# alehdaghi/vq-vae-2-pytorch

Hardware: AMD Instinct MI355X
Metric: images/sec VQ-VAE-2 256px train step (higher is better)
Workload: dtype f32; 1 GPU; configs[1]: 256x256 FFHQ-shaped synthetic, default two-level VQ-VAE-2, batch 32/GPU; global_batch=32, image=256, n_embed=512, parallelism=dp1

## Files before the change

### include/vq2.h

```cpp
#ifndef VQ2_H
#define VQ2_H

#include <stddef.h>
#include <stdint.h>

#ifdef __cplusplus
extern "C" {
#endif

#define VQ2_OK 0
#define VQ2_ERR_INVALID 1
#define VQ2_ERR_UNSUPPORTED 2
#define VQ2_ERR_WORKSPACE 3
#define VQ2_ERR_LAUNCH 4

typedef void *vq2_stream_t;

#define VQ2_API_VERSION 12

int vq2_version(void);
const char *vq2_last_error(void);

int vq2_prof_enable(int level);
int vq2_prof_report(char *buf, size_t cap);

typedef struct vq2_conv_desc {
    int32_t N, H, W, Ci;
    int32_t Co;
    int32_t KH, KW, stride, pad;
    int32_t transposed;
    int32_t ldx, ldy;
    int32_t Cir, Cor;
} vq2_conv_desc;

#define VQ2_RELU_IN 1
#define VQ2_RELU_OUT 2

#define VQ2_PACK_FWD 0
#define VQ2_PACK_DGRAD 1
int vq2_pack_weight(const vq2_conv_desc *d, int which, const float *w, float *packed, vq2_stream_t stream);

typedef struct vq2_pack_job {
    const float *w;
    float *packed;
    int64_t offset;
    int64_t numel;
    int32_t Or, Ir, Op, Ip, KH, KW, mode, reserved;
} vq2_pack_job;
int vq2_pack_job_init(const vq2_conv_desc *d, int which, const float *w, float *packed, vq2_pack_job *job);
int vq2_pack_weights_batched(const vq2_pack_job *jobs_dev, int32_t njobs, int64_t total, vq2_stream_t stream);

// ... 7 lines not shown

size_t vq2_resblock_w2_workspace_bytes(int32_t N, int32_t H, int32_t W, int32_t C, int32_t Cm);
int vq2_resblock_bwd_data(int32_t N, int32_t H, int32_t W, int32_t C, int32_t Cm, const float *g, int32_t ldg,
                          const float *r, int32_t ldr, const float *x, int32_t ldx, const float *w2d, const float *w1d,
                          float *dh, int32_t lddh, float *dx, int32_t lddx, void *w2_ws, vq2_stream_t stream);

int vq2_conv_dgrad(const vq2_conv_desc *d, const float *dy, const float *wp, const float *mask, int32_t ldmask,
                   const float *residual, int32_t ldres, float *dx, int32_t lddx, vq2_stream_t stream);
#define VQ2_MASK_AFTER_RESIDUAL 4
int vq2_conv_dgrad_ex(const vq2_conv_desc *d, int flags, const float *dy, const float *wp, const float *mask,
                      int32_t ldmask, const float *residual, int32_t ldres, float *dx, int32_t lddx,
                      vq2_stream_t stream);

size_t vq2_conv_wgrad_workspace_bytes(const vq2_conv_desc *d);
int vq2_conv_wgrad(const vq2_conv_desc *d, int flags, const float *x, const float *dy, float *dw, float *db, void *ws,
                   size_t ws_bytes, vq2_stream_t stream);

typedef struct vq2_wgrad_job {
    const float *ws;
    float *dw;
    const float *bias_ws;
    float *db;
    int64_t unit_offset;
    int32_t O, I, Or, Ir, taps, S, n_units_w, n_units_b;
    int32_t swapped;
    int32_t bias_splits;
} vq2_wgrad_job;
int vq2_conv_wgrad_partial(const vq2_conv_desc *d, int flags, const float *x, const float *dy, float *db, void *ws,
                           size_t ws_bytes, vq2_stream_t stream);
int vq2_wgrad_job_init(const vq2_conv_desc *d, const void *ws, float *dw, float *db, vq2_wgrad_job *job);
int vq2_wgrad_reduce_batched(const vq2_wgrad_job *jobs_dev, int32_t njobs, int64_t total_units, vq2_stream_t stream);
int vq2_resblock_w2_job_init(int32_t N, int32_t H, int32_t W, int32_t C, int32_t Cm, const void *ws, float *dw, float *db,
                             vq2_wgrad_job *job);

size_t vq2_colsum_workspace_bytes(int64_t rows, int32_t C);
int vq2_colsum(const float *dy, int64_t rows, int32_t C, int32_t ld, float *db, void *ws, size_t ws_bytes,
               vq2_stream_t stream);

int vq2_nchw_to_nhwc(const float *src, float *dst, int32_t N, int32_t C, int32_t H, int32_t W, int32_t ld,
                     vq2_stream_t stream);
int vq2_nhwc_to_nchw(const float *src, float *dst, int32_t N, int32_t C, int32_t H, int32_t W, int32_t ld,
                     vq2_stream_t stream);

#define VQ2_U8_HWC 0
#define VQ2_U8_CHW 1
int vq2_u8_to_nhwc4(const uint8_t *src, int layout, int32_t N, int32_t C, int32_t Hs, int32_t Ws, int32_t y0,
                    int32_t x0, int32_t H, int32_t W, const float *lut ,
                    float *dst , vq2_stream_t stream);
int vq2_nhwc_to_u8(const float *src, int32_t ld, int32_t N, int32_t C, int32_t H, int32_t W,
                   const float *inv_s , const float *mean , uint8_t *dst, int layout,
                   int32_t Hc, int32_t Wc, int64_t pitch, int32_t cols, int32_t pad, int64_t image_pitch, vq2_stream_t stream);
int vq2_relu_bwd(const float *dy, int32_t lddy, const float *y, int32_t ldy, float *g, int32_t ldg, int64_t pixels,
                 int32_t C, vq2_stream_t stream);
int vq2_slice_copy(const float *src, int32_t lds, float *dst, int32_t ldd, int64_t pixels, int32_t C,
                   int accumulate, vq2_stream_t stream);

int vq2_vq_prepare(const float *embed, float *embedT, float *enorm, int32_t D, int32_t K, vq2_stream_t stream);
size_t vq2_vq_fwd_workspace_floats(int64_t M, int32_t D, int32_t K);
int vq2_vq_fwd(const float *x, int32_t ldx, const float *embed, const float *embedT, const float *enorm, int64_t M,
               int32_t D, int32_t K, int64_t *idx, float *out, int32_t ldo, float *ws, vq2_stream_t stream);
size_t vq2_vq_stats_workspace_bytes(int64_t M, int32_t D, int32_t K);
int vq2_vq_stats(const float *x, int32_t ldx, const int64_t *idx, int64_t M, int32_t D, int32_t K, float *counts,
                 float *sumsT, void *ws, size_t ws_bytes, vq2_stream_t stream);
int vq2_vq_loss(const float *loss_partial, int64_t M, int32_t D, float *diff, vq2_stream_t stream);
int vq2_vq_bwd(const float *g_out, int32_t ldg, const float *g_diff, const float *x, int32_t ldx,
               const int64_t *idx, const float *embedT, int64_t M, int32_t D, int32_t K, float *dx, int32_t lddx,
// ... 158 lines not shown
```

### vq-vae-2-pytorch_amd/_lib.py

```python
import ctypes as C
import os

_HERE = os.path.dirname(os.path.abspath(__file__))
LIB_PATH = os.environ.get("VQ2_LIB") or os.path.join(_HERE, "libvq2.so")

c_f32p = C.c_void_p
c_stream = C.c_void_p


class ConvDesc(C.Structure):
    _fields_ = [(n, C.c_int32) for n in
                ("N", "H", "W", "Ci", "Co", "KH", "KW", "stride", "pad", "transposed", "ldx", "ldy", "Cir", "Cor")]


class ConvGeom(C.Structure):
    _fields_ = [(n, C.c_int32) for n in
                ("N", "H", "W", "Ci", "Co", "KH", "KW", "pad_top", "pad_left", "ldx", "ldy", "Cir", "Cor", "reserved")]


class PackJob(C.Structure):
    _fields_ = [("w", C.c_void_p), ("packed", C.c_void_p), ("offset", C.c_int64), ("numel", C.c_int64)] + \
               [(n, C.c_int32) for n in ("Or", "Ir", "Op", "Ip", "KH", "KW", "mode", "reserved")]


# ... 15 lines not shown

class WnEntry(C.Structure):
    _fields_ = [("v_off", C.c_int64), ("g_off", C.c_int64), ("w_off", C.c_int64)] + \
               [(n, C.c_int32) for n in ("rows", "cols", "kh", "kw", "mask_from", "row_start")]


def _load():
    if not os.path.exists(LIB_PATH):
        raise ImportError(
            f"{LIB_PATH} not found: build it with `python -c 'import __graft_entry__ as g; g.build()'` "
            "(vq-vae-2-pytorch_amd/csrc/build.sh).  There is no CPU or eager fallback for this path.")
    import torch
    lib = C.CDLL(LIB_PATH)
    P, I32, I64, SZ, F, D = C.c_void_p, C.c_int32, C.c_int64, C.c_size_t, C.c_float, C.c_double
    DP = C.POINTER(ConvDesc)
    GP = C.POINTER(ConvGeom)
    U64 = C.c_uint64
    sig = {
        "vq2_version": (C.c_int, []),
        "vq2_last_error": (C.c_char_p, []),
        "vq2_prof_enable": (C.c_int, [C.c_int]),
        "vq2_prof_report": (C.c_int, [C.c_char_p, SZ]),
        "vq2_pack_weight": (C.c_int, [DP, C.c_int, P, P, P]),
        "vq2_pack_job_init": (C.c_int, [DP, C.c_int, P, P, C.POINTER(PackJob)]),
        "vq2_pack_weights_batched": (C.c_int, [P, I32, I64, P]),
        "vq2_conv_fwd": (C.c_int, [DP, C.c_int, P, P, P, P, I32, P, P]),
        "vq2_conv_dgrad": (C.c_int, [DP, P, P, P, I32, P, I32, P, I32, P]),
        "vq2_conv_dgrad_ex": (C.c_int, [DP, C.c_int, P, P, P, I32, P, I32, P, I32, P]),
        "vq2_conv_wgrad_workspace_bytes": (SZ, [DP]),
        "vq2_conv_wgrad": (C.c_int, [DP, C.c_int, P, P, P, P, P, SZ, P]),
        "vq2_conv_wgrad_partial": (C.c_int, [DP, C.c_int, P, P, P, P, SZ, P]),
        "vq2_wgrad_job_init": (C.c_int, [DP, P, P, P, C.POINTER(WgradJob)]),
        "vq2_wgrad_reduce_batched": (C.c_int, [P, I32, I64, P]),
        "vq2_colsum_workspace_bytes": (SZ, [I64, I32]),
        "vq2_colsum": (C.c_int, [P, I64, I32, I32, P, P, SZ, P]),
        "vq2_nchw_to_nhwc": (C.c_int, [P, P, I32, I32, I32, I32, I32, P]),
        "vq2_nhwc_to_nchw": (C.c_int, [P, P, I32, I32, I32, I32, I32, P]),
        "vq2_u8_to_nhwc4": (C.c_int, [P, C.c_int, I32, I32, I32, I32, I32, I32, I32, I32, P, P, P]),
        "vq2_nhwc_to_u8": (C.c_int, [P, I32, I32, I32, I32, I32, C.POINTER(F), C.POINTER(F), P, C.c_int, I32, I32, I64, I32,
                                     I32, I64, P]),
        "vq2_sse_workspace_bytes": (SZ, [I32, I32, I32, I32]),
        "vq2_sse_per_image": (C.c_int, [P, P, I32, I32, I32, I32, P, P, SZ, P]),
        "vq2_index_hist": (C.c_int, [P, I64, I32, P, P, P]),
        "vq2_eval_accumulate": (C.c_int, [P, I32, I64, P, P, P]),
        "vq2_image_metrics_workspace_bytes": (SZ, [I32, I32, I32, I32]),
        "vq2_image_metrics": (C.c_int, [P, I32, P, I32, I32, I32, I32, I32, C.POINTER(F), C.POINTER(F), P, P, P, SZ, P]),
        "vq2_image_metrics_accumulate": (C.c_int, [P, P, I32, P, P, P]),
        "vq2_relu_bwd": (C.c_int, [P, I32, P, I32, P, I32, I64, I32, P]),
        "vq2_resblock_supported": (C.c_int, [I32, I32]),
        "vq2_resblock_bwd_data": (C.c_int, [I32, I32, I32, I32, I32, P, I32, P, I32, P, I32, P, P, P, I32, P, I32, P, P]),
        "vq2_resblock_w2_workspace_bytes": (SZ, [I32, I32, I32, I32, I32]),
        "vq2_resblock_w2_job_init": (C.c_int, [I32, I32, I32, I32, I32, P, P, P, C.POINTER(WgradJob)]),
        "vq2_resblock_fwd": (C.c_int, [I32, I32, I32, I32, I32, C.c_int, P, I32, P, P, P, P, P, I32, P, I32, P]),
        "vq2_slice_copy": (C.c_int, [P, I32, P, I32, I64, I32, C.c_int, P]),
        "vq2_vq_prepare": (C.c_int, [P, P, P, I32, I32, P]),
        "vq2_vq_fwd_workspace_floats": (SZ, [I64, I32, I32]),
        "vq2_vq_fwd": (C.c_int, [P, I32, P, P, P, I64, I32, I32, P, P, I32, P, P]),
        "vq2_vq_stats_workspace_bytes": (SZ, [I64, I32, I32]),
        "vq2_vq_stats": (C.c_int, [P, I32, P, I64, I32, I32, P, P, P, SZ, P]),
        "vq2_vq_loss": (C.c_int, [P, I64, I32, P, P]),
        "vq2_vq_bwd": (C.c_int, [P, I32, P, P, I32, P, P, I64, I32, I32, P, I32, P]),
        "vq2_vq_ema_update": (C.c_int, [P, P, P, P, P, I32, I32, D, D, P, P]),
        "vq2_vq_ema_update_prepare": (C.c_int, [P, P, P, P, P, I32, I32, D, D, P, P, P, P]),
        "vq2_vq_gather": (C.c_int, [P, P, I64, I32, I32, P, I32, P]),
        "vq2_instnorm_stats": (C.c_int, [P, I32, I32, I64, I32, D, P, P, P]),
        "vq2_adain_fwd": (C.c_int, [P, I32, P, P, P, I32, I64, I32, C.c_int, P, I32, P]),
# ... 78 lines not shown
```

### vq-vae-2-pytorch_amd/csrc/vq2_wgrad.hip

```cpp
#include "vq2_conv.h"

namespace vq2 {

struct WgradParams {
    const float *x;
    const float *g;
    float *ws;
    float *bias_ws;
    int bias_taps;
    int bias_nslots;
    int N, H, W, I, ldx;
    int Ho, Wo, O, ldg;
    int KH, KW, stride, pad_h, pad_w;
    int K, M;
    int rows_per_split;
    int relu_x, relu_g;
};

constexpr int WG_BKR = 32;

constexpr int rows_per_pass(int c4) {
    int r = 32;
    while (r * c4 > 256) r >>= 1;
    return r;
// ... 648 lines not shown
        const int t = (is_bias ? lu - j.n_units_w : lu) * 32 + lane;
        float s0 = 0.f, s1 = 0.f, s2 = 0.f, s3 = 0.f;
        if (t < limit) {
            int z = g;
            for (; z + 24 < nsplit; z += 32) {
                s0 += src[(size_t)z * total + t];
                s1 += src[(size_t)(z + 8) * total + t];
                s2 += src[(size_t)(z + 16) * total + t];
                s3 += src[(size_t)(z + 24) * total + t];
            }
            for (; z < nsplit; z += 8) s0 += src[(size_t)z * total + t];
        }
        part[g][lane] = (s0 + s1) + (s2 + s3);
        __syncthreads();
        if (g == 0 && t < limit) {
            float s = part[0][lane];
#pragma unroll
            for (int q = 1; q < 8; ++q) s += part[q][lane];
            if (is_bias) {
                j.db[t] = s;
            } else {
                const int o = t / K, k = t - o * K;
                const int tap = k / j.I, i = k - tap * j.I;
                if (o < j.Or && i < j.Ir) {
                    if (j.swapped & 1) j.dw[((size_t)i * j.Or + o) * j.taps + (j.taps - 1 - tap)] = s;
                    else j.dw[((size_t)o * j.Ir + i) * j.taps + tap] = s;
                }
            }
        }
        __syncthreads();
    }
}

enum WgradRole { WGRAD_PLAIN, WGRAD_EXCHANGED, WGRAD_CONVT };
enum WgradFamily { WGRAD_GEN, WGRAD_FAST, WGRAD_WINO };

struct WgradPlan {
    int role, family;
    int wino;
    int tile;
    int O, I, K, M, S, rows_per_split;
    int Or, Ir;
    int bias_taps, bias_nslots, bias_splits;
    size_t bias_floats;
    int mode;
    long ext_x, ext_g;
};

static WgradParams wgrad_operands(const ConvGeo *d, int role) {
    WgradParams P{};
    P.N = d->N; P.KH = d->KH; P.KW = d->KW; P.stride = d->stride; P.pad_h = d->pad_h; P.pad_w = d->pad_w;
    P.H = d->H; P.W = d->W; P.Ho = d->H; P.Wo = d->W;
    P.ldx = role == WGRAD_PLAIN ? d->ldx : d->ldy;
    P.ldg = role == WGRAD_PLAIN ? d->ldy : d->ldx;
    if (role == WGRAD_PLAIN) { P.Ho = out_hw(d).h; P.Wo = out_hw(d).w; }
    else if (role == WGRAD_CONVT) { P.H = 2 * d->H; P.W = 2 * d->W; }
    else { P.stride = 1; P.pad_h = P.pad_w = d->KH - 1 - d->pad_h; }
    return P;
}

template <int WM, int WN, int MT, int NT>
static int launch_wgrad(const WgradPlan &pl, const WgradParams &P, hipStream_t s) {
    constexpr int BMO = WM * MT * 32, BNK = WN * NT * 32;
    const bool rx = P.relu_x, rg = P.relu_g;
    void (*kern)(const WgradParams) = nullptr;
    if (pl.family == WGRAD_GEN) kern = wgrad_kernel<WM, WN, MT, NT>;
    else if (pl.family == WGRAD_FAST)
        kern = rx ? wgrad_fast_kernel<WM, WN, MT, NT, true, false>
                  : rg ? wgrad_fast_kernel<WM, WN, MT, NT, false, true> : wgrad_fast_kernel<WM, WN, MT, NT, false, false>;
    else if constexpr (BMO == 128 && BNK == 128) {
        if (pl.wino == 1) kern = rx ? wgrad_fast_kernel<WM, WN, MT, NT, true, false, 1> : wgrad_fast_kernel<WM, WN, MT, NT, false, false, 1>;
        if (pl.wino == 2)
            kern = rx ? wgrad_fast_kernel<WM, WN, MT, NT, true, false, 2>
                      : rg ? wgrad_fast_kernel<WM, WN, MT, NT, false, true, 2> : wgrad_fast_kernel<WM, WN, MT, NT, false, false, 2>;
    } else if constexpr (BMO == 128 && BNK == 96) {
        if (pl.wino == 3) kern = rg ? wgrad_fast_kernel<WM, WN, MT, NT, false, true, 3> : wgrad_fast_kernel<WM, WN, MT, NT, false, false, 3>;
    }
    if (!kern) return set_error(VQ2_ERR_INVALID, "conv_wgrad: the %d x %d tile has no Winograd mode %d", BMO, BNK, pl.wino);
    const size_t lds = (size_t)2 * WG_BKR * (BMO + BNK) * sizeof(float);
// ... 69 lines not shown
            if (best < 0 || work < best) { best = work; p.tile = c; }
        }
    }
    if (wino && p.role == WGRAD_EXCHANGED && d->KH == 3 && d->pad_h == 1 && p.I == 32 && p.O % 128 == 0 &&
        (d->W % 64 == 0 || (d->W == 32 && d->H % 2 == 0))) {
        p.wino = 3;
        p.K = 4 * 96;
        p.M = p.M / 2;
        p.tile = wgrad_tile_of(128, 96);
    }
    const int bmo = WGRAD_TILES[p.tile].bmo, bnk = WGRAD_TILES[p.tile].bnk;
    const int tiles = ((p.K + bnk - 1) / bnk) * ((p.O + bmo - 1) / bmo);
    const int lds = 2 * WG_BKR * (bmo + bnk) * 4;
    int per_cu = (160 * 1024) / lds;
    if (per_cu > 4) per_cu = 4;
    int S = (256 * per_cu) / tiles;
    const int max_s = (p.M + 255) / 256;
    if (S > max_s) S = max_s;
    if (S < 1) S = 1;
    int rps = (p.M + S - 1) / S;
    rps = (rps + 31) / 32 * 32;
    p.S = (p.M + rps - 1) / rps;
    p.rows_per_split = rps;
    p.ext_x = (long)d->N * v.H * v.W * v.ldx;
    p.ext_g = (long)p.M * v.ldg;
    const bool fast_ok = fast && v.Wo % WG_BKR == 0 && p.rows_per_split % WG_BKR == 0 && p.ext_x < FAST_REACH && p.ext_g < FAST_REACH;
    p.family = p.wino ? WGRAD_WINO : fast_ok ? WGRAD_FAST : WGRAD_GEN;
    if (p.wino == 2 && d->transposed) { p.bias_taps = 1; p.bias_nslots = 4; }
    else if (p.role == WGRAD_EXCHANGED) { p.bias_taps = 1 << ((d->KH / 2) * d->KW + d->KW / 2); p.bias_nslots = 1; }
    else if (d->transposed) { p.bias_taps = (1 << 5) | (1 << 6) | (1 << 9) | (1 << 10); p.bias_nslots = 4; }
    p.bias_floats = p.bias_taps ? (size_t)p.S * p.bias_nslots * p.I : (size_t)p.S * p.O;
    p.bias_splits = p.bias_taps ? p.S * p.bias_nslots : 0;
    p.mode = (p.role == WGRAD_EXCHANGED) | (p.wino << 1);
    return p;
}

static size_t wgrad_ws_bytes(const WgradPlan &p) { return ((size_t)p.S * p.O * p.K + p.bias_floats) * sizeof(float); }

static int wgrad_params(const ConvGeo *d, const WgradPlan &p, int flags, const float *x, const float *dy, float *db, void *ws,
                        WgradParams &P) {
    VQ2_REQUIRE(p.ext_x < (1L << 31) && p.ext_g < (1L << 31), "conv_wgrad: tensor exceeds 2^31 elements");
    const bool plain = p.role == WGRAD_PLAIN;
    const int relu = (flags & VQ2_RELU_IN) != 0;
    P = wgrad_operands(d, p.role);
    P.x = plain ? x : dy; P.relu_x = plain ? relu : 0;
    P.g = plain ? dy : x; P.relu_g = plain ? 0 : relu;
    P.ws = static_cast<float *>(ws);
    P.bias_ws = db ? P.ws + (size_t)p.S * p.O * p.K : nullptr;
    P.bias_taps = p.bias_taps; P.bias_nslots = p.bias_nslots;
    P.O = p.O; P.I = p.I; P.K = p.K; P.M = p.M; P.rows_per_split = p.rows_per_split;
    return VQ2_OK;
}

static const char *wgrad_label(const WgradPlan &p, const WgradTile &t, const ConvGeo *d) {
    const char *form = p.wino == 3 ? "swwino" : p.role == WGRAD_EXCHANGED ? "sw" : p.wino == 1 ? "wino" : p.wino == 2 ? "wino4" : "";
    return prof_label("wgrad<%dx%d>%s|O=%d,K=%d,M=%d,S=%d,k%d,%s", t.bmo, t.bnk, form, p.O, p.K, p.M, p.S, d->KH,
                      p.family == WGRAD_GEN ? "gen" : "fast");
}

constexpr int CS_MAX_BLOCKS = 512;

static inline int64_t cs_rows_per_block(int64_t rows) {
    int64_t rpb = (rows + CS_MAX_BLOCKS - 1) / CS_MAX_BLOCKS;
    return rpb < 256 ? 256 : rpb;
}

__global__ __launch_bounds__(256) void colsum_partial_kernel(const float *__restrict__ x, int64_t rows, int C, int ld,
                                                             int64_t rpb, float *__restrict__ part) {
    extern __shared__ __attribute__((aligned(16))) float red[];
    const int C4 = C / 4;
    const int nrg = 256 / C4 > 0 ? 256 / C4 : 1;
    const int64_t r0 = (int64_t)blockIdx.x * rpb;
    const int64_t r1 = r0 + rpb < rows ? r0 + rpb : rows;
    for (int cbase = 0; cbase < C4; cbase += 256) {
        const int c4 = cbase + (int)(threadIdx.x % (C4 < 256 ? C4 : 256));
        const int rg = threadIdx.x / (C4 < 256 ? C4 : 256);
        float4 a = make_float4(0.f, 0.f, 0.f, 0.f);
        if (rg < nrg && c4 < C4) {
            for (int64_t r = r0 + rg; r < r1; r += nrg) {
                const float4 v = *reinterpret_cast<const float4 *>(x + r * ld + c4 * 4);
                a.x += v.x; a.y += v.y; a.z += v.z; a.w += v.w;
            }
            *reinterpret_cast<float4 *>(red + (size_t)rg * C + c4 * 4) = a;
        }
        __syncthreads();
        for (int c = threadIdx.x; c < C; c += 256) {
            if (c / 4 >= cbase && c / 4 < cbase + 256) {
                float s = 0.f;
                for (int g = 0; g < nrg; ++g) s += red[(size_t)g * C + c];
                part[(size_t)blockIdx.x * C + c] = s;
// ... 99 lines not shown
    if (int e = wgrad_params(d, p, flags, x, dy, db, ws, P)) return e;
    hipStream_t s = to_stream(stream);
    const WgradTile &tile = WGRAD_TILES[p.tile];
    const ConvWork work = conv_work(d, 0, 0);
    ProfScope prof(prof_enabled() ? wgrad_label(p, tile, d) : "wgrad", work.flops, work.bytes, s);
    if (int e = tile.launch(p, P, s)) return e;
    if (!reduce) return VQ2_OK;
    vq2_wgrad_job j;
    wgrad_job_init_impl(d, p, ws, dw, db, &j);
    const int total = p.O * p.K;
    const int blocks = (total + 31) / 32 < 4096 ? (total + 31) / 32 : 4096;
    hipLaunchKernelGGL(wgrad_reduce_kernel, dim3(blocks), dim3(256), 0, s, j.ws, j.dw, j.O, j.I, j.Or, j.Ir, j.taps, j.S,
                       j.bias_ws, j.db, j.swapped, j.bias_splits);
    return check_launch("wgrad_reduce_kernel");
}

extern "C" int vq2_conv_wgrad(const vq2_conv_desc *d, int flags, const float *x, const float *dy, float *dw, float *db,
                              void *ws, size_t ws_bytes, vq2_stream_t stream) {
    return wgrad_impl(d, flags, x, dy, dw, db, ws, ws_bytes, stream, true);
}
extern "C" int vq2_conv_wgrad_partial(const vq2_conv_desc *d, int flags, const float *x, const float *dy, float *db,
                                      void *ws, size_t ws_bytes, vq2_stream_t stream) {
    return wgrad_impl(d, flags, x, dy, nullptr, db, ws, ws_bytes, stream, false);
}
extern "C" int vq2_convg_wgrad(const vq2_conv_geom *d, int flags, const float *x, const float *dy, float *dw, float *db,
                               void *ws, size_t ws_bytes, vq2_stream_t stream) {
    return wgrad_impl(d, flags, x, dy, dw, db, ws, ws_bytes, stream, true);
}
extern "C" int vq2_convg_wgrad_partial(const vq2_conv_geom *d, int flags, const float *x, const float *dy, float *db,
                                       void *ws, size_t ws_bytes, vq2_stream_t stream) {
    return wgrad_impl(d, flags, x, dy, nullptr, db, ws, ws_bytes, stream, false);
}

template <class Desc>
static int wgrad_job_entry(const Desc *d, const void *ws, float *dw, float *db, vq2_wgrad_job *job) {
    ConvGeo g;
    if (int e = entry_geo(d, "wgrad_job_init", g)) return e;
    VQ2_REQUIRE(ws && dw && job, "wgrad_job_init: null pointer");
    VQ2_REQUIRE(!g.same || (g.N > 0 && g.H > 0 && g.W > 0 && g.Ci > 0 && g.Co > 0), "wgrad_job_init: non-positive dims");
    if (int e = check_forms()) return e;
    wgrad_job_init_impl(&g, plan_wgrad(&g), ws, dw, db, job);
    return VQ2_OK;
}

extern "C" int vq2_wgrad_job_init(const vq2_conv_desc *d, const void *ws, float *dw, float *db, vq2_wgrad_job *job) {
    return wgrad_job_entry(d, ws, dw, db, job);
}
extern "C" int vq2_convg_wgrad_job_init(const vq2_conv_geom *d, const void *ws, float *dw, float *db, vq2_wgrad_job *job) {
    return wgrad_job_entry(d, ws, dw, db, job);
}

extern "C" int vq2_wgrad_reduce_batched(const vq2_wgrad_job *jobs_dev, int32_t njobs, int64_t total_units,
                                        vq2_stream_t stream) {
    VQ2_REQUIRE(jobs_dev && njobs > 0 && total_units > 0, "wgrad_reduce_batched: bad arguments");
    const unsigned blocks = (unsigned)(total_units < 8192 ? total_units : 8192);
    hipLaunchKernelGGL(wgrad_reduce_batched_kernel, dim3(blocks), dim3(256), 0, to_stream(stream), jobs_dev, njobs,
                       total_units);
    return check_launch("wgrad_reduce_batched_kernel");
}

extern "C" size_t vq2_colsum_workspace_bytes(int64_t rows, int32_t C) {
    if (rows <= 0 || C <= 0) return 0;
    const int64_t rpb = cs_rows_per_block(rows);
    return (size_t)((rows + rpb - 1) / rpb) * C * sizeof(float);
}

// ... 9 lines not shown
```

### vq-vae-2-pytorch_amd/ops.py

```python
from dataclasses import dataclass
from types import SimpleNamespace
import contextlib
import ctypes as C
import os

import torch
from torch.autograd import Function

from ._lib import lib, check, AttnDesc, ConvDesc, ConvGeom, OneHotDesc, PackJob, WgradJob, WnEntry

VQ2_RELU_IN = 1
VQ2_RELU_OUT = 2
VQ2_MASK_AFTER_RESIDUAL = 4
PACK_FWD = 0
PACK_DGRAD = 1



def _stream():
    return C.c_void_p(torch.cuda.current_stream().cuda_stream)


_THIS_STREAM = contextlib.nullcontext()

# ... 207 lines not shown
    check(_abi(spec).fwd(C.byref(d), flags, _p(x), _p(wp), _p(bias), _p(residual), ldres, _p(out), _stream()),
          "conv_fwd")
    return out


def conv_dgrad(spec, xshape, dy, weight, mask=None, residual=None, out=None, mask_after=False):
    n, h, w, _ = xshape
    if out is None:
        out = torch.empty((n, h, w, spec.ci), device=dy.device, dtype=torch.float32)
    d = _desc(spec, n, h, w, spec.ci, ld_of(dy))
    wp = packed_weight(spec, weight, PACK_DGRAD)
    check(_abi(spec).dgrad(C.byref(d), VQ2_MASK_AFTER_RESIDUAL if mask_after else 0, _p(dy), _p(wp), _p(mask),
                                ld_of(mask) if mask is not None else 0, _p(residual),
                                ld_of(residual) if residual is not None else 0, _p(out), ld_of(out), _stream()),
          "conv_dgrad")
    return out


def _grad_slot(param):
    slot = getattr(param, "_vq2_grad", None) if param is not None else None
    if slot is not None and (not param.is_leaf or param.grad is None):
        return slot.view_as(slot)
    return None if param is None else torch.empty_like(param, memory_format=torch.contiguous_format)


class WgradBatch:

    def __init__(self):
        self.entries = {}
        self.order = []
        self.tables = {}
        self.dirty = True

    def launch(self, spec, x, dy, relu_in, weight, bias, want_db, side):
        n, h, w, _ = x.shape
        key = (id(weight), n, h, w, ld_of(x), ld_of(dy), relu_in)
        d = _desc(spec, n, h, w, ld_of(x), ld_of(dy))
        ent = self.entries.get(key)
        if ent is None:
            nbytes = _abi(spec).wgrad_workspace_bytes(C.byref(d))
            ws = torch.empty(max(nbytes // 4, 4), device=x.device, dtype=torch.float32)
            dw = weight._vq2_grad
            db = bias._vq2_grad if (bias is not None and want_db) else None
            job = WgradJob()
            check(_abi(spec).wgrad_job_init(C.byref(d), _p(ws), _p(dw), _p(db), C.byref(job)), "wgrad_job_init")
            ent = {"ws": ws, "nbytes": nbytes, "job": job, "dw": dw, "db": db, "used": False}
            self.entries[key] = ent
            self.dirty = True
        on_side = n * h * w <= WGRAD_STREAM_MAX_PIXELS
        if on_side:
            side.wait_event(torch.cuda.current_stream().record_event())
        with (torch.cuda.stream(side) if on_side else _THIS_STREAM):
            check(_abi(spec).wgrad_partial(C.byref(d), VQ2_RELU_IN if relu_in else 0, _p(x), _p(dy), _p(ent["db"]),
                                             _p(ent["ws"]), ent["nbytes"], _stream()), "conv_wgrad_partial")
        if on_side:
            x.record_stream(side)
            dy.record_stream(side)
        if not ent["used"]:
            ent["used"] = True
            self.order.append(key)
        dw, db = ent["dw"], ent["db"]
        return dw.view_as(dw), (None if db is None else db.view_as(db))

    def resblock_w2(self, n, h, w, c, cm, weight, bias):
        key = (id(weight), n, h, w, "rbw2")
        ent = self.entries.get(key)
        if ent is None:
            nbytes = lib.vq2_resblock_w2_workspace_bytes(n, h, w, c, cm)
            ws = torch.empty(max(nbytes // 4, 4), device=weight.device, dtype=torch.float32)
            dw, db = weight._vq2_grad, bias._vq2_grad
            job = WgradJob()
            check(lib.vq2_resblock_w2_job_init(n, h, w, c, cm, _p(ws), _p(dw), _p(db), C.byref(job)), "resblock_w2_job_init")
            ent = {"ws": ws, "nbytes": nbytes, "job": job, "dw": dw, "db": db, "used": False}
            self.entries[key] = ent
            self.dirty = True
        if not ent["used"]:
            ent["used"] = True
            self.order.append(key)
        return ent["ws"], ent["dw"].view_as(ent["dw"]), ent["db"].view_as(ent["db"])

    def flush(self):
        if not self.order:
            return
        sig = tuple(self.order)
        if self.dirty:
            self.tables = {}
            self.dirty = False
        tab = self.tables.get(sig)
        if tab is None:
            import numpy as np
            arr = (WgradJob * len(self.order))()
            off = 0
            for i, key in enumerate(self.order):
                job = self.entries[key]["job"]
                job.unit_offset = off
                arr[i] = job
                off += job.n_units_w + job.n_units_b
            raw = np.frombuffer(bytes(arr), dtype=np.uint8).copy()
            tab = (torch.from_numpy(raw).to(self.entries[self.order[0]]["ws"].device), off)
            self.tables[sig] = tab
        check(lib.vq2_wgrad_reduce_batched(_p(tab[0]), len(self.order), tab[1], _stream()), "wgrad_reduce_batched")
        for key in self.order:
            self.entries[key]["used"] = False
        self.order = []


class StepContext:

    def __init__(self, wgrad_stream):
        self.batch = WgradBatch()
        self.stream = wgrad_stream
        self.active = False


def _step_ctx(weight):
    ctx = getattr(weight, "_vq2_ctx", None)
    return ctx if (ctx is not None and ctx.active) else None


WGRAD_STREAM_MAX_PIXELS = 40000


def conv_wgrad(spec, x, dy, relu_in, weight, bias=None, want_dw=True, want_db=True):
    n, h, w, _ = x.shape
    d = _desc(spec, n, h, w, ld_of(x), ld_of(dy))
    nbytes = _abi(spec).wgrad_workspace_bytes(C.byref(d))
    sc = _step_ctx(weight)
    if sc is not None and getattr(weight, "_vq2_grad", None) is not None and weight.grad is None and \
            (bias is None or (getattr(bias, "_vq2_grad", None) is not None and bias.grad is None)) and \
            (bias is None or bias.numel() == spec.cout):
        dw, db = sc.batch.launch(spec, x, dy, relu_in, weight, bias, want_db, sc.stream)
        return (dw if want_dw else None), db
    dw = _grad_slot(weight)
    db = _grad_slot(bias) if (bias is not None and want_db) else None
    side = None
    if sc is not None and getattr(weight, "_vq2_grad", None) is not None and dw.data_ptr() == weight._vq2_grad.data_ptr():
        side = sc.stream
        side.wait_event(torch.cuda.current_stream().record_event())
    with (torch.cuda.stream(side) if side is not None else _THIS_STREAM):
        ws = torch.empty(max(nbytes // 4, 4), device=x.device, dtype=torch.float32)
        check(_abi(spec).wgrad(C.byref(d), VQ2_RELU_IN if relu_in else 0, _p(x), _p(dy), _p(dw), _p(db), _p(ws), nbytes,
                                 _stream()), "conv_wgrad")
    if side is not None:
        x.record_stream(side)
        dy.record_stream(side)
    return (dw if want_dw else None), db


def relu_bwd(dy, y):
    n, h, w, c = dy.shape
    g = torch.empty((n, h, w, c), device=dy.device, dtype=torch.float32)
    check(lib.vq2_relu_bwd(_p(dy), ld_of(dy), _p(y), ld_of(y), _p(g), c, n * h * w, c, _stream()), "relu_bwd")
    return g


def add_(a, b, alpha=1.0):
    a, b = packed(a), packed(b)
    out = torch.empty_like(a)
    check(lib.vq2_axpby(_p(a), _p(b), float(alpha), _p(out), a.numel(), _stream()), "axpby")
    return out


class NchwToNhwc(Function):
# ... 196 lines not shown
        return True

    def take(self):
        t, self.tensor, self.closed = self.tensor, None, True
        return t


class ConvFn(Function):

    @staticmethod
    def forward(ctx, x, weight, bias, residual, spec, flags, out, grad_stash=None, mask_input=False, premasked=False):
        ctx.grad_stash, ctx.mask_input, ctx.premasked = grad_stash, mask_input, premasked
        x = as_nhwc(x)
        if residual is not None:
            residual = as_nhwc(residual)
        y = conv_forward(spec, x, weight, bias, flags, residual, out)
        ctx.spec, ctx.flags = spec, flags
        ctx.has_res = residual is not None
        ctx.has_bias = bias is not None
        ctx.save_for_backward(x, weight, y if (flags & VQ2_RELU_OUT) else None, bias)
        if out is not None:
            y = y.view_as(y)
        return y

    @staticmethod
    def backward(ctx, dy):
        x, weight, y, bias = ctx.saved_tensors
        spec, flags = ctx.spec, ctx.flags
        g = as_nhwc(dy)
        if (flags & VQ2_RELU_OUT) and not ctx.premasked:
            g = relu_bwd(g, y)
        relu_in = bool(flags & VQ2_RELU_IN)
        dx = dw = db = dres = None
        if ctx.needs_input_grad[0]:
            other = ctx.grad_stash.take() if ctx.grad_stash is not None else None
            dx = conv_dgrad(spec, x.shape, g, weight, mask=x if (relu_in or ctx.mask_input) else None, residual=other,
                            mask_after=ctx.mask_input)
        if ctx.needs_input_grad[1] or (ctx.has_bias and ctx.needs_input_grad[2]):
            dw, db = conv_wgrad(spec, x, g, relu_in, weight, bias, ctx.needs_input_grad[1],
                                ctx.has_bias and ctx.needs_input_grad[2])
        if ctx.has_res and ctx.needs_input_grad[3]:
            dres = g
        return dx, dw, db, dres, None, None, None, None, None, None


def conv_op(x, weight, bias, spec, relu_in=False, relu_out=False, residual=None, out=None, grad_stash=None,
            mask_input=False, premasked=False):
    flags = (VQ2_RELU_IN if relu_in else 0) | (VQ2_RELU_OUT if relu_out else 0)
    if grad_stash is not None and relu_in and not mask_input:
        grad_stash.closed = True
        grad_stash = None
    return ConvFn.apply(x, weight, bias, residual, spec, flags, out, grad_stash, mask_input, premasked)


_FORMS = os.environ.get("VQ2_FORMS", "all")
if _FORMS not in ("all", "direct", "general"):
    raise ValueError(f"VQ2_FORMS={_FORMS!r}: expected all, direct or general")

RESBLOCK_FUSED = [_FORMS != "general"]


class ResBlockFn(Function):

    @staticmethod
    def forward(ctx, x, w1, b1, w2, b2, spec1, spec2, relu_out, out, premasked=False):
        ctx.premasked = premasked
# ... 842 lines not shown
```

Baseline: 5448 images/s.

## Fuse dgrad and wgrad of final 64->3 transposed conv into one-pass kernel

Adds a kernel for the final conv-transpose layer (64 to at most 4 channels, k4 s2 p1) that reads the input activation and output gradient tiles once and computes both the weight-gradient partials and the input gradient (with the ReLU mask applied) in the same pass using MFMA. This removes one full read of the large full-resolution gradient and of the input, and one kernel launch, compared with separate dgrad and wgrad. The Python backward takes the fused path when the layer qualifies, and the deferred wgrad reduction is still batched. Tradeoffs are higher register and LDS pressure and the loss of wgrad overlap on the side stream for this layer.

```diff
diff --git a/include/vq2.h b/include/vq2.h
--- a/include/vq2.h
+++ b/include/vq2.h
@@ -16,7 +16,7 @@
 
 typedef void *vq2_stream_t;
 
-#define VQ2_API_VERSION 12
+#define VQ2_API_VERSION 13
 
 int vq2_version(void);
 const char *vq2_last_error(void);
@@ -90,6 +90,10 @@
 int vq2_wgrad_reduce_batched(const vq2_wgrad_job *jobs_dev, int32_t njobs, int64_t total_units, vq2_stream_t stream);
 int vq2_resblock_w2_job_init(int32_t N, int32_t H, int32_t W, int32_t C, int32_t Cm, const void *ws, float *dw, float *db,
                              vq2_wgrad_job *job);
+
+int vq2_recon_bwd_supported(const vq2_conv_desc *d, int32_t lddx);
+int vq2_recon_bwd(const vq2_conv_desc *d, const float *x, const float *dy, const float *wp, float *dx, int32_t lddx,
+                  float *dw, float *db, void *ws, size_t ws_bytes, vq2_stream_t stream);
 
 size_t vq2_colsum_workspace_bytes(int64_t rows, int32_t C);
 int vq2_colsum(const float *dy, int64_t rows, int32_t C, int32_t ld, float *db, void *ws, size_t ws_bytes,
diff --git a/vq-vae-2-pytorch_amd/_lib.py b/vq-vae-2-pytorch_amd/_lib.py
--- a/vq-vae-2-pytorch_amd/_lib.py
+++ b/vq-vae-2-pytorch_amd/_lib.py
@@ -71,6 +71,8 @@
         "vq2_conv_wgrad_partial": (C.c_int, [DP, C.c_int, P, P, P, P, SZ, P]),
         "vq2_wgrad_job_init": (C.c_int, [DP, P, P, P, C.POINTER(WgradJob)]),
         "vq2_wgrad_reduce_batched": (C.c_int, [P, I32, I64, P]),
+        "vq2_recon_bwd_supported": (C.c_int, [DP, I32]),
+        "vq2_recon_bwd": (C.c_int, [DP, P, P, P, P, I32, P, P, P, SZ, P]),
         "vq2_colsum_workspace_bytes": (SZ, [I64, I32]),
         "vq2_colsum": (C.c_int, [P, I64, I32, I32, P, P, SZ, P]),
         "vq2_nchw_to_nhwc": (C.c_int, [P, P, I32, I32, I32, I32, I32, P]),
diff --git a/vq-vae-2-pytorch_amd/csrc/vq2_wgrad.hip b/vq-vae-2-pytorch_amd/csrc/vq2_wgrad.hip
--- a/vq-vae-2-pytorch_amd/csrc/vq2_wgrad.hip
+++ b/vq-vae-2-pytorch_amd/csrc/vq2_wgrad.hip
@@ -704,6 +704,171 @@
     }
 }
 
+namespace rb {
+constexpr int LD = 68;
+constexpr int PIX = 2 * WG_BKR;
+constexpr int COOB = 0x7F000000;
+constexpr long REACH = COOB / 4;
+}
+
+struct ReconBwdParams {
+    const float *x;
+    const float *dy;
+    const float *wp;
+    float *dx;
+    float *ws;
+    float *bias_ws;
+    int N, H, W, ldx, ldy, lddx;
+    int M, rows_per_split;
+};
+
+template <bool C4>
+__global__ __launch_bounds__(256, C4 ? 3 : 4) void recon_bwd_kernel(const ReconBwdParams P) {
+    using namespace rb;
+    __shared__ __attribute__((aligned(16))) float Gs[PIX * LD];
+    __shared__ __attribute__((aligned(16))) float Xs[PIX * LD];
+    const int tid = threadIdx.x, lane = tid & 63, wave = tid >> 6;
+    const int l31 = lane & 31, h = lane >> 5;
+    const int wm = wave >> 1, wn = wave & 1;
+    const int dj = wave & 1, dc = wave >> 1;
+    const int split = xcd_remap(blockIdx.x, gridDim.x);
+    const int m_begin = split * P.rows_per_split;
+    const int m_end = min(P.M, m_begin + P.rows_per_split);
+
+    const __amdgpu_buffer_rsrc_t rx = __builtin_amdgcn_make_buffer_rsrc(const_cast<float *>(P.x), 0, P.M * P.ldx * 4, RSRC_FLAGS);
+    const __amdgpu_buffer_rsrc_t rdy = __builtin_amdgcn_make_buffer_rsrc(const_cast<float *>(P.dy), 0, 4 * P.M * P.ldy * 4, RSRC_FLAGS);
+    const __amdgpu_buffer_rsrc_t rw = __builtin_amdgcn_make_buffer_rsrc(const_cast<float *>(P.wp), 0, 64 * 64 * 4, RSRC_FLAGS);
+    const __amdgpu_buffer_rsrc_t rdx = __builtin_amdgcn_make_buffer_rsrc(P.dx, 0, P.M * P.lddx * 4, RSRC_FLAGS);
+
+    float4 wf[8];
+#pragma unroll
+    for (int k8 = 0; k8 < 8; ++k8)
+        wf[k8] = as_f4(__builtin_amdgcn_raw_buffer_load_b128(rw, ((dj * 32 + l31) * 64 + 8 * k8 + 4 * h) * 4, 0, 0));
+
+    const int g_r = tid >> 4, g_c = (tid & 15) * 4;
+    const int x_r = tid >> 2, kh = tid & 3;
+    int xn, xho, xwo;
+    {
+        const int m = m_begin + x_r, hw = P.H * P.W;
+        xn = m / hw;
+        const int r = m - xn * hw;
+        xho = r / P.W;
+        xwo = r - xho * P.W;
+    }
+    u32x4 rgv[4], rxv[4];
+    auto load_pixels = [&](int mbase) {
+#pragma unroll
+        for (int j = 0; j < 4; ++j) {
+            const int m = mbase + g_r + 16 * j;
+            rgv[j] = __builtin_amdgcn_raw_buffer_load_b128(rx, m < m_end ? (m * P.ldx + g_c) * 4 : COOB, 0, 0);
+        }
+        const int ih = 2 * xho - 1 + kh, iw0 = 2 * xwo - 1;
+        const bool rv = mbase + x_r < m_end && (unsigned)ih < (unsigned)(2 * P.H);
+        const int base = ((xn * 2 * P.H + ih) * 2 * P.W + iw0) * P.ldy * 4;
+#pragma unroll
+        for (int kw = 0; kw < 4; ++kw)
+            rxv[kw] = __builtin_amdgcn_raw_buffer_load_b128(rdy, (rv && (unsigned)(iw0 + kw) < (unsigned)(2 * P.W)) ? base + kw * P.ldy * 4 : COOB, 0, 0);
+        xwo += PIX;
+        while (xwo >= P.W) {
+            xwo -= P.W;
+            if (++xho == P.H) { xho = 0; ++xn; }
+        }
+    };
+    auto store_pixels = [&]() {
+#pragma unroll
+        for (int j = 0; j < 4; ++j)
+            *reinterpret_cast<float4 *>(Gs + (g_r + 16 * j) * LD + g_c) = relu4(as_f4(rgv[j]));
+#pragma unroll
+        for (int kw = 0; kw < 4; ++kw)
+            *reinterpret_cast<float4 *>(Xs + x_r * LD + (kh * 4 + kw) * 4) = as_f4(rxv[kw]);
+    };
+
+    f32x16 acc;
+#pragma unroll
+    for (int r = 0; r < 16; ++r) acc[r] = 0.f;
+    int bx_col = -1;
+    if (P.bias_ws != nullptr && tid < 64) {
+        const int tap = tid >> 2;
+        const unsigned taps = (1u << 5) | (1u << 6) | (1u << 9) | (1u << 10);
+        if ((taps >> tap) & 1) bx_col = __popc(taps & ((1u << tap) - 1u)) * 4 + (tid & 3);
+    }
+    const bool do_bias_x = bx_col >= 0;
+    float bsum = 0.f;
+
+    const int nchunks = (m_end - m_begin + WG_BKR - 1) / WG_BKR;
+    const int niter = (nchunks + 1) / 2;
+    if (niter > 0) load_pixels(m_begin);
+    for (int it = 0; it < niter; ++it) {
+        const int mbase = m_begin + it * PIX;
+        const bool two = 2 * it + 1 < nchunks;
+        store_pixels();
+        __syncthreads();
+        if (it + 1 < niter) load_pixels(mbase + PIX);
+        if (do_bias_x) {
+            for (int cc = 0; cc < (two ? 2 : 1); ++cc) {
+                const float *xcol = Xs + cc * WG_BKR * LD + tid;
+                float s0 = 0.f, s1 = 0.f;
+#pragma unroll
+                for (int r = 0; r < WG_BKR; r += 2) { s0 += xcol[r * LD]; s1 += xcol[(r + 1) * LD]; }
+                bsum += s0 + s1;
+            }
+        }
+        for (int cc = 0; cc < (two ? 2 : 1); ++cc) {
+            const float *gs = Gs + (cc * WG_BKR + h) * LD + wm * 32 + l31;
+            const float *xs = Xs + (cc * WG_BKR + h) * LD + wn * 32 + l31;
+            float fa[2], fb[2];
+            fa[0] = gs[0]; fb[0] = xs[0];
+#pragma unroll
+            for (int kk = 0; kk < WG_BKR / 2; ++kk) {
+                const int cur = kk & 1, nxt = cur ^ 1;
+                if (kk + 1 < WG_BKR / 2) { fa[nxt] = gs[(kk + 1) * 2 * LD]; fb[nxt] = xs[(kk + 1) * 2 * LD]; }
+                acc = __builtin_amdgcn_mfma_f32_32x32x2f32(fa[cur], fb[cur], acc, 0, 0, 0);
+                __builtin_amdgcn_sched_group_barrier(0x100, 2, 0);
+                __builtin_amdgcn_sched_group_barrier(0x008, 1, 0);
+            }
+        }
+        if (dc == 0 || two) {
+            f32x16 dacc;
+#pragma unroll
+            for (int r = 0; r < 16; ++r) dacc[r] = 0.f;
+            const float *xp = Xs + (dc * WG_BKR + l31) * LD + 4 * h;
+            float4 bq[2];
+            bq[0] = *reinterpret_cast<const float4 *>(xp);
+#pragma unroll
+            for (int k8 = 0; k8 < 8; ++k8) {
+                const int cur = k8 & 1, nxt = cur ^ 1;
+                if (k8 + 1 < 8) bq[nxt] = *reinterpret_cast<const float4 *>(xp + 8 * (k8 + 1));
+                const float4 b = bq[cur];
+                dacc = __builtin_amdgcn_mfma_f32_32x32x2f32(wf[k8].x, b.x, dacc, 0, 0, 0);
+                dacc = __builtin_amdgcn_mfma_f32_32x32x2f32(wf[k8].y, b.y, dacc, 0, 0, 0);
+                dacc = __builtin_amdgcn_mfma_f32_32x32x2f32(wf[k8].z, b.z, dacc, 0, 0, 0);
+                if (C4) dacc = __builtin_amdgcn_mfma_f32_32x32x2f32(wf[k8].w, b.w, dacc, 0, 0, 0);
+                __builtin_amdgcn_sched_group_barrier(0x100, 1, 0);
+                __builtin_amdgcn_sched_group_barrier(0x008, C4 ? 4 : 3, 0);
+            }
+            const int m = mbase + dc * WG_BKR + l31;
+            const bool pv = m < m_end;
+            const float *gp = Gs + (dc * WG_BKR + l31) * LD + 32 * dj + 4 * h;
+#pragma unroll
+            for (int g = 0; g < 4; ++g) {
+                const float4 mk = *reinterpret_cast<const float4 *>(gp + 8 * g);
+                float4 o = make_float4(dacc[4 * g] + 0.f, dacc[4 * g + 1] + 0.f, dacc[4 * g + 2] + 0.f, dacc[4 * g + 3] + 0.f);
+                o.x = mk.x > 0.f ? o.x : 0.f; o.y = mk.y > 0.f ? o.y : 0.f; o.z = mk.z > 0.f ? o.z : 0.f; o.w = mk.w > 0.f ? o.w : 0.f;
+                u32x4 u;
+                u.x = __float_as_uint(o.x); u.y = __float_as_uint(o.y); u.z = __float_as_uint(o.z); u.w = __float_as_uint(o.w);
+                __builtin_amdgcn_raw_buffer_store_b128(u, rdx, pv ? (m * P.lddx + 32 * dj + 8 * g + 4 * h) * 4 : COOB, 0, 0);
+            }
+        }
+        __syncthreads();
+    }
+
+    if (do_bias_x) P.bias_ws[(size_t)split * 16 + bx_col] = bsum;
+    float *slab = P.ws + (size_t)split * 64 * 64;
+    const int k = wn * 32 + l31, ob = wm * 32 + 4 * h;
+#pragma unroll
+    for (int r = 0; r < 16; ++r) slab[(ob + (r & 3) + 8 * (r >> 2)) * 64 + k] = acc[r];
+}
+
 enum WgradRole { WGRAD_PLAIN, WGRAD_EXCHANGED, WGRAD_CONVT };
 enum WgradFamily { WGRAD_GEN, WGRAD_FAST, WGRAD_WINO };
 
@@ -717,6 +882,7 @@
     size_t bias_floats;
     int mode;
     long ext_x, ext_g;
+    bool recon;
 };
 
 static WgradParams wgrad_operands(const ConvGeo *d, int role) {
@@ -852,6 +1018,8 @@
     p.bias_floats = p.bias_taps ? (size_t)p.S * p.bias_nslots * p.I : (size_t)p.S * p.O;
     p.bias_splits = p.bias_taps ? p.S * p.bias_nslots : 0;
     p.mode = (p.role == WGRAD_EXCHANGED) | (p.wino << 1);
+    p.recon = fast && p.role == WGRAD_CONVT && !p.wino && p.O == 64 && p.I == 4 && bmo == 64 && bnk == 64 &&
+              p.ext_x < rb::REACH && p.ext_g < rb::REACH;
     return p;
 }
 
@@ -876,6 +1044,10 @@
     const char *form = p.wino == 3 ? "swwino" : p.role == WGRAD_EXCHANGED ? "sw" : p.wino == 1 ? "wino" : p.wino == 2 ? "wino4" : "";
     return prof_label("wgrad<%dx%d>%s|O=%d,K=%d,M=%d,S=%d,k%d,%s", t.bmo, t.bnk, form, p.O, p.K, p.M, p.S, d->KH,
                       p.family == WGRAD_GEN ? "gen" : "fast");
+}
+
+static const char *recon_bwd_label(const WgradPlan &p, const WgradTile &t, const ConvGeo *d) {
+    return prof_label("wgrad<%dx%d>recon_bwd|O=%d,K=%d,M=%d,S=%d,k%d,fused", t.bmo, t.bnk, p.O, p.K, p.M, p.S, d->KH);
 }
 
 constexpr int CS_MAX_BLOCKS = 512;
@@ -1041,6 +1213,59 @@
     return wgrad_impl(d, flags, x, dy, nullptr, db, ws, ws_bytes, stream, false);
 }
 
+static bool recon_bwd_ok(const ConvGeo *d, const WgradPlan &p, int32_t lddx) {
+    return p.recon && d->transposed && d->KH == 4 && d->KW == 4 && d->stride == 2 && d->pad_h == 1 && lddx >= d->Ci &&
+           lddx % 4 == 0 && (long)p.M * lddx < rb::REACH;
+}
+
+extern "C" int vq2_recon_bwd_supported(const vq2_conv_desc *d, int32_t lddx) {
+    if (!d || check_forms() || d->N <= 0 || d->H <= 0 || d->W <= 0 || d->Ci <= 0 || d->Co <= 0 || d->KH <= 0 || d->KW <= 0 ||
+        d->ldx < d->Ci || d->ldy < d->Co || d->ldx % 4 || d->ldy % 4)
+        return 0;
+    const ConvGeo g = geo_of(d);
+    return recon_bwd_ok(&g, plan_wgrad(&g), lddx) ? 1 : 0;
+}
+
+extern "C" int vq2_recon_bwd(const vq2_conv_desc *desc, const float *x, const float *dy, const float *wp, float *dx,
+                             int32_t lddx, float *dw, float *db, void *ws, size_t ws_bytes, vq2_stream_t stream) {
+    VQ2_REQUIRE(desc, "recon_bwd: null pointer");
+    const ConvGeo g = geo_of(desc);
+    const ConvGeo *d = &g;
+    VQ2_REQUIRE(x && dy && wp && dx && ws, "recon_bwd: null pointer");
+    if (int e = check_forms()) return e;
+    VQ2_REQUIRE(d->N > 0 && d->H > 0 && d->W > 0 && d->Ci > 0 && d->Co > 0 && d->Ci % 4 == 0 && d->Co % 4 == 0, "recon_bwd: bad dims");
+    VQ2_REQUIRE(d->ldx >= d->Ci && d->ldy >= d->Co && d->ldx % 4 == 0 && d->ldy % 4 == 0, "recon_bwd: bad strides");
+    VQ2_REQUIRE(aligned16(x) && aligned16(dy) && aligned16(wp) && aligned16(dx) && aligned16(ws),
+                "recon_bwd: pointers must be 16-byte aligned");
+    const WgradPlan p = plan_wgrad(d);
+    if (!recon_bwd_ok(d, p, lddx))
+        return set_error(VQ2_ERR_UNSUPPORTED, "recon_bwd: not a layer of the one-pass kernel (ask vq2_recon_bwd_supported): "
+                         "conv-transpose 64 -> <= 4 channels, k4 s2 p1, tensors below %d bytes", rb::COOB);
+    VQ2_REQUIRE(ws_bytes >= wgrad_ws_bytes(p), "recon_bwd: workspace too small");
+    ReconBwdParams P{};
+    P.x = x; P.dy = dy; P.wp = wp; P.dx = dx;
+    P.ws = static_cast<float *>(ws);
+    P.bias_ws = db ? P.ws + (size_t)p.S * p.O * p.K : nullptr;
+    P.N = d->N; P.H = d->H; P.W = d->W; P.ldx = d->ldx; P.ldy = d->ldy; P.lddx = lddx;
+    P.M = p.M; P.rows_per_split = p.rows_per_split;
+    hipStream_t s = to_stream(stream);
+    {
+        const ConvWork work = conv_work(d, 1, 0);
+        ProfScope prof(prof_enabled() ? recon_bwd_label(p, WGRAD_TILES[p.tile], d) : "recon_bwd", 2.0 * work.flops, work.bytes, s);
+        const bool c4 = !(real_co(d) > 0 && real_co(d) <= 3);
+        hipLaunchKernelGGL(c4 ? recon_bwd_kernel<true> : recon_bwd_kernel<false>, dim3(p.S), dim3(256), 0, s, P);
+        if (int e = check_launch("recon_bwd_kernel")) return e;
+    }
+    if (!dw) return VQ2_OK;
+    vq2_wgrad_job j;
+    wgrad_job_init_impl(d, p, ws, dw, db, &j);
+    const int total = p.O * p.K;
+    const int blocks = (total + 31) / 32 < 4096 ? (total + 31) / 32 : 4096;
+    hipLaunchKernelGGL(wgrad_reduce_kernel, dim3(blocks), dim3(256), 0, s, j.ws, j.dw, j.O, j.I, j.Or, j.Ir, j.taps, j.S,
+                       j.bias_ws, j.db, j.swapped, j.bias_splits);
+    return check_launch("wgrad_reduce_kernel");
+}
+
 template <class Desc>
 static int wgrad_job_entry(const Desc *d, const void *ws, float *dw, float *db, vq2_wgrad_job *job) {
     ConvGeo g;
diff --git a/vq-vae-2-pytorch_amd/ops.py b/vq-vae-2-pytorch_amd/ops.py
--- a/vq-vae-2-pytorch_amd/ops.py
+++ b/vq-vae-2-pytorch_amd/ops.py
@@ -263,7 +263,7 @@
         self.tables = {}
         self.dirty = True
 
-    def launch(self, spec, x, dy, relu_in, weight, bias, want_db, side):
+    def _entry(self, spec, x, dy, relu_in, weight, bias, want_db):
         n, h, w, _ = x.shape
         key = (id(weight), n, h, w, ld_of(x), ld_of(dy), relu_in)
         d = _desc(spec, n, h, w, ld_of(x), ld_of(dy))
@@ -275,9 +275,28 @@
             db = bias._vq2_grad if (bias is not None and want_db) else None
             job = WgradJob()
             check(_abi(spec).wgrad_job_init(C.byref(d), _p(ws), _p(dw), _p(db), C.byref(job)), "wgrad_job_init")
-            ent = {"ws": ws, "nbytes": nbytes, "job": job, "dw": dw, "db": db, "used": False}
+            ent = {"ws": ws, "nbytes": nbytes, "job": job, "dw": dw, "db": db, "used": False, "key": key}
             self.entries[key] = ent
             self.dirty = True
+        return d, ent
+
+    def _used(self, ent):
+        if not ent["used"]:
+            ent["used"] = True
+            self.order.append(ent["key"])
+        dw, db = ent["dw"], ent["db"]
+        return dw.view_as(dw), (None if db is None else db.view_as(db))
+
+    def recon_bwd(self, spec, x, dy, weight, bias, want_db, dx):
+        d, ent = self._entry(spec, x, dy, True, weight, bias, want_db)
+        wp = packed_weight(spec, weight, PACK_DGRAD)
+        check(lib.vq2_recon_bwd(C.byref(d), _p(x), _p(dy), _p(wp), _p(dx), ld_of(dx), None, _p(ent["db"]), _p(ent["ws"]),
+                                ent["nbytes"], _stream()), "recon_bwd")
+        return self._used(ent)
+
+    def launch(self, spec, x, dy, relu_in, weight, bias, want_db, side):
+        n, h, w, _ = x.shape
+        d, ent = self._entry(spec, x, dy, relu_in, weight, bias, want_db)
         on_side = n * h * w <= WGRAD_STREAM_MAX_PIXELS
         if on_side:
             side.wait_event(torch.cuda.current_stream().record_event())
@@ -287,11 +306,7 @@
         if on_side:
             x.record_stream(side)
             dy.record_stream(side)
-        if not ent["used"]:
-            ent["used"] = True
-            self.order.append(key)
-        dw, db = ent["dw"], ent["db"]
-        return dw.view_as(dw), (None if db is None else db.view_as(db))
+        return self._used(ent)
 
     def resblock_w2(self, n, h, w, c, cm, weight, bias):
         key = (id(weight), n, h, w, "rbw2")
@@ -352,14 +367,44 @@
 WGRAD_STREAM_MAX_PIXELS = 40000
 
 
+def _deferred(sc, spec, weight, bias):
+    return sc is not None and getattr(weight, "_vq2_grad", None) is not None and weight.grad is None and \
+        (bias is None or (getattr(bias, "_vq2_grad", None) is not None and bias.grad is None)) and \
+        (bias is None or bias.numel() == spec.cout)
+
+
+def recon_bwd_supported(spec, x, dy):
+    if spec.is_geom or not spec.transposed:
+        return False
+    n, h, w, _ = x.shape
+    d = _desc(spec, n, h, w, ld_of(x), ld_of(dy))
+    return bool(lib.vq2_recon_bwd_supported(C.byref(d), spec.ci))
+
+
+def recon_bwd(spec, x, dy, weight, bias=None, want_db=True):
+    n, h, w, _ = x.shape
+    dx = torch.empty((n, h, w, spec.ci), device=dy.device, dtype=torch.float32)
+    sc = _step_ctx(weight)
+    if _deferred(sc, spec, weight, bias):
+        dw, db = sc.batch.recon_bwd(spec, x, dy, weight, bias, want_db, dx)
+        return dx, dw, db
+    d = _desc(spec, n, h, w, ld_of(x), ld_of(dy))
+    nbytes = _abi(spec).wgrad_workspace_bytes(C.byref(d))
+    dw = _grad_slot(weight)
+    db = _grad_slot(bias) if (bias is not None and want_db) else None
+    ws = torch.empty(max(nbytes // 4, 4), device=x.device, dtype=torch.float32)
+    wp = packed_weight(spec, weight, PACK_DGRAD)
+    check(lib.vq2_recon_bwd(C.byref(d), _p(x), _p(dy), _p(wp), _p(dx), ld_of(dx), _p(dw), _p(db), _p(ws), nbytes, _stream()),
+          "recon_bwd")
+    return dx, dw, db
+
+
 def conv_wgrad(spec, x, dy, relu_in, weight, bias=None, want_dw=True, want_db=True):
     n, h, w, _ = x.shape
     d = _desc(spec, n, h, w, ld_of(x), ld_of(dy))
     nbytes = _abi(spec).wgrad_workspace_bytes(C.byref(d))
     sc = _step_ctx(weight)
-    if sc is not None and getattr(weight, "_vq2_grad", None) is not None and weight.grad is None and \
-            (bias is None or (getattr(bias, "_vq2_grad", None) is not None and bias.grad is None)) and \
-            (bias is None or bias.numel() == spec.cout):
+    if _deferred(sc, spec, weight, bias):
         dw, db = sc.batch.launch(spec, x, dy, relu_in, weight, bias, want_db, sc.stream)
         return (dw if want_dw else None), db
     dw = _grad_slot(weight)
@@ -622,6 +667,10 @@
             g = relu_bwd(g, y)
         relu_in = bool(flags & VQ2_RELU_IN)
         dx = dw = db = dres = None
+        if ctx.needs_input_grad[0] and ctx.needs_input_grad[1] and relu_in and not ctx.mask_input and \
+                ctx.grad_stash is None and recon_bwd_supported(spec, x, g):
+            dx, dw, db = recon_bwd(spec, x, g, weight, bias, ctx.has_bias and ctx.needs_input_grad[2])
+            return dx, dw, db, (g if ctx.has_res and ctx.needs_input_grad[3] else None), None, None, None, None, None, None
         if ctx.needs_input_grad[0]:
             other = ctx.grad_stash.take() if ctx.grad_stash is not None else None
             dx = conv_dgrad(spec, x.shape, g, weight, mask=x if (relu_in or ctx.mask_input) else None, residual=other,
```

Measured after the change: 5487 images/s, median of 6. About the same (+0.7%).
